# CurryChen77/RIFT

Measured on AMD Instinct MI355X. Metric: policy-update scenes/sec (256-scene RIFT update steps on a 4096-scene replay), higher is better.
Workload: dtype bf16; 1 GPU; BASELINE configs[2]/[3]: full rift_pluto CBV policy, 4096-scene synthetic replay (64 agents x 21 steps, 20 polygons x 3 x 20 pts, R~U{1..6} x 120 ref pts, 12 modes), RIFT loss, pi_head trainable; per_gpu_batch=256, global_batch=256, replay_scenes_per_gpu=4096, parallelism=dp1, train_mode=dropout+droppath+state-dropout, BN batch stats

## Files before the change

rift_amd/csrc/engine.hip:

```cpp
#include <hip/hip_runtime.h>
#include <math.h>
#include <stdio.h>
#include <stdlib.h>
#include <string.h>

#include <set>
#include <cmath>
#include <string>
#include <unordered_map>
#include <dlfcn.h>
#include <vector>

#include "../../include/rift_hip.h"
#include "adv.h"
#include "gemm.h"
#include "kernels.h"
#include "loss.h"
#include "nat_l0w.h"
#include "nat_l1w.h"
#include "enc_fused.h"
#include "enc_fused.h"
#include "dec_w.h"
#include "dec_kv.h"
#include "nat_l2w.h"
#include "enc_w.h"
#include "pe_w.h"
#include "fo_w.h"
#include "pe_fused.h"
#include "fourier_fused.h"
#include "critic.h"
#include "fpn_fused.h"
#include "ego_fused.h"
#include "front.h"
#include "heads_fused.h"
#include "pi_fused.h"
#include "rollout.h"
#include "tick_multi.h"

#define ENC_NW 8

using namespace RIFT_NS;

namespace {

struct Param { void* data; int64_t numel; int ndim; int64_t shape[4]; };

struct PW {
  void* bf = nullptr; float* f32 = nullptr; const float* bias = nullptr;
  int N = 0, K = 0, Kp = 0, Npad = 0;
  void* hid = nullptr;
};

struct Tap { float* p; int64_t numel; };

}

struct RiftCtx {
  int opfmt = 0;
  int device = 0;
  std::string err;
  std::unordered_map<std::string, Param> params;
  std::unordered_map<std::string, PW> pw;
  std::vector<void*> owned;
  struct WConst { float* p = nullptr; bool ready = false; };
// ... 12 lines not shown
  float* ro_raw = nullptr; size_t ro_cap = 0;
  char* tick_scratch = nullptr; size_t tick_cap = 0;
  bool dry = false;
  hipStream_t stream = nullptr;
  std::unordered_map<std::string, Tap> taps;
  float* last_qfinal = nullptr; float* last_hpi = nullptr; float* last_prob = nullptr;
  uint8_t* last_rkpm = nullptr; int last_bs = 0, last_R = 0;
  double* l_S = nullptr; double* l_cnt = nullptr; float* l_dz = nullptr; float* l_partial = nullptr;
  size_t l_cap_bs = 0, l_cap_rows = 0, l_cap_wg = 0;
  float* ego_w = nullptr; float* ego_b = nullptr;
  bool nat_fused = true; int gemm_dbg = 0;
  unsigned short* l0w_img = nullptr; float* l0w_par = nullptr;
  unsigned short* encw_img = nullptr; float* encw_par = nullptr;
  unsigned short* l2w_img = nullptr; float* l2w_par = nullptr;
  unsigned short* l1w_img = nullptr; float* l1w_par = nullptr;
  unsigned short* enc_wqkv[4] = {nullptr, nullptr, nullptr, nullptr};
  float* enc_bqkv[4] = {nullptr, nullptr, nullptr, nullptr};
  int* enc_idx = nullptr; bool enc_fused = true;
  int poison_lds = -1;
  struct { std::string delay_label; long long delay_ticks = 0; int pe_ts = -1, pew_dbg = 0, pew_ts = 0, nat_ts = 0, enc_ts = 0, dec_ts = 0, dec_dbg = 0, poison_arena = -1; } dg;
  hipEvent_t param_event = nullptr;
  bool dec_fused = true;
  bool two_streams = true; bool nat_on_main = true; bool nat_compact = true; bool pe_live = true; bool pe_pack = true; bool tok_fused = false; bool keep_tokens = false; bool front_fused = false; bool front_ego = false; bool ego_nofit = false;
  hipStream_t prep_stream = nullptr; bool prep_set = false; hipEvent_t ev_prep = nullptr; int side_gate = 0;
  hipEvent_t ev_join2 = nullptr; bool nat_aside = true; int join_once = -1;
  hipStream_t side = nullptr; bool side_owned = false; hipEvent_t ev_fork = nullptr, ev_join = nullptr;
  bool fo_w = true; unsigned short* fow_img[3] = {nullptr, nullptr, nullptr}; float* fow_par[3] = {nullptr, nullptr, nullptr};
  bool pe_w = true; unsigned short* pew_img[2] = {nullptr, nullptr};
  unsigned short* decw_img = nullptr; float* decw_par = nullptr;
  double* clip_part = nullptr;
  struct Dp { bool on = false; int off = 0, gbs = 0; double* xchg = nullptr; long long len = 0; RiftExchangeFn fn = nullptr; void* user = nullptr; } dp;
  int* nonfinite = nullptr;
  unsigned long long* rk_pub[RIFT_DEFER_SLOTS] = {}; int rk_cap[RIFT_DEFER_SLOTS] = {}; unsigned int rk_epoch[RIFT_DEFER_SLOTS] = {};
  bool rank_fault = false;
  bool enc112 = true;
  bool rank_in_prep = true;
  void* comm = nullptr; int comm_rank = 0, comm_world = 1;
  float* cr_buf = nullptr; size_t cr_cap = 0; double* cr_part = nullptr;
  bool pe_fused = true; bool fo_fused = true; int nat_grid = 256; bool fpn_fused = true; bool ego_fused = true; bool heads_fused = true; bool pi_fused = true;
  bool loaded = false;
  bool prof_on = false; double prof_flops = 0.0; bool prof_shapes = false;
  std::set<std::string> prof_names;
  std::vector<hipEvent_t> prof_pool; size_t prof_used = 0;
  struct Rec { const char* label; hipEvent_t e0, e1; double flops; };
  std::vector<Rec> prof_recs;
};

static void prof_events(RiftCtx* c, hipEvent_t* e0, hipEvent_t* e1) {
  while (c->prof_pool.size() < c->prof_used + 2) { hipEvent_t e; (void)hipEventCreate(&e); c->prof_pool.push_back(e); }
  *e0 = c->prof_pool[c->prof_used++]; *e1 = c->prof_pool[c->prof_used++];
}
static void prof_push(RiftCtx* c, const char* label, hipEvent_t e0, hipEvent_t e1, double flops) {
  c->prof_recs.push_back(RiftCtx::Rec{label, e0, e1, flops});
}

#define HIPCHK(ctx, expr)                                                                 \
  do {                                                                                    \
    hipError_t e__ = (expr);                                                              \
    if (e__ != hipSuccess) {                                                              \
      (ctx)->err = std::string(#expr) + ": " + hipGetErrorString(e__);                    \
      return RIFT_ERR_HIP;                                                                \
    }                                                                                     \
  } while (0)

namespace {

// ... 702 lines not shown
    g.gbias = h.x0p; g.gb_div = R * M; g.gb_mod = 0;
    gemm(c, g, c->pw[PD + ".cat_x_proj.q"], h.fp32);
    PW w; w.N = 128; w.K = 128; w.Kp = 128; w.Npad = 128;
    w.f32 = (float*)fptr(c, PD + ".pi_head.mlp.0.weight"); w.bias = fptr(c, PD + ".pi_head.mlp.0.bias");
    gemm(c, mk(h.QF, 128, nQ, w, h.Hpi, 128), w, true);
    launch(c, "pi_tail_kernel", pi_tail_kernel, dim3(cdiv(nQ, 4)), dim3(256), 0, (const float*)h.Hpi, nQ, M, fptr(c, PD + ".pi_head.mlp.1.weight"),
           fptr(c, PD + ".pi_head.mlp.1.bias"), fptr(c, PD + ".pi_head.mlp.3.weight"), fptr(c, PD + ".pi_head.mlp.3.bias"),
           (const uint8_t*)h.r_kpm, 1e-5f, h.prob, c->nonfinite);
  }
  tap(c, "q_final", h.QF, (int64_t)nQ * 128);
  if (h.need_traj && !h.fp32 && c->heads_fused) {
    const std::string nm3[3] = {PD + ".loc_head", PD + ".yaw_head", PD + ".vel_head"};
    heads3_fused(f, h.QF, 128, nQ, 0, 0, 0, nm3, h.traj);
  } else if (h.need_traj) {
    const char* nm[3] = {"loc_head", "yaw_head", "vel_head"};
    for (int i = 0; i < 3; ++i) {
      const PW& w0 = c->pw[PD + "." + nm[i] + ".mlp.0"];
      const PW& w3 = c->pw[PD + "." + nm[i] + ".mlp.3"];
      float* T = h.oT[i];
      gemm(c, mk(h.QF, 128, nQ, w0, T, w0.N), w0, h.fp32);
      GemmP g = mk(T, w0.N, nQ, w3, h.o3[i], 160);
      g.pro = PRO_LN; g.pg = fptr(c, PD + "." + nm[i] + ".mlp.1.weight"); g.pb = fptr(c, PD + "." + nm[i] + ".mlp.1.bias"); g.pro_relu = 1;
      gemm(c, g, w3, h.fp32);
    }
    launch(c, "interleave_traj_kernel", interleave_traj_kernel, dim3(cdiv((long long)nQ * 480, 256)), dim3(256), 0, (const float*)h.o3[0], (const float*)h.o3[1],
           (const float*)h.o3[2], nQ, h.traj);
  }
  if (!c->dry) {
    c->last_qfinal = h.QF; c->last_hpi = h.Hpi; c->last_prob = h.prob; c->last_rkpm = h.r_kpm; c->last_bs = h.bs; c->last_R = h.R;
  }
  return RIFT_OK;
}

int forward_impl(RiftCtx* c, const RiftFeatureBatch* B, const RiftOutputs* out, int flags, uint32_t seed) {
  Fwd f;
  f.c = c; f.train = (flags & RIFT_F_TRAIN) != 0; f.drop = f.train && !(flags & RIFT_F_NO_DROP);
  f.fp32 = (flags & RIFT_F_FP32) != 0; f.need_traj = (flags & RIFT_F_NEED_TRAJ) != 0;
  f.bn_update = f.train && !(flags & RIFT_F_NO_BN_UPDATE); f.seed = seed;
  const int bs = B->bs, A = B->A, Mp = B->Mp, R = B->R, S = B->S, T = B->T;
  const int N = A + Mp + S, M = 12;
  const int nA = bs * A, nP = bs * Mp, nL = bs * R, nQ = nL * M, nT = bs * N;
  const std::string HE = "agent_encoder.history_encoder";

  (void)A_alloc<float>(c, 64);
  float* F9 = A_alloc<float>(c, (size_t)nA * 20 * 9 + 64);
  uint8_t* valid_agent = A_alloc<uint8_t>(c, nA);
  const bool nat_compact = c->nat_compact && c->nat_fused && !f.fp32 && c->fpn_fused;
  uint8_t* hist_agent = nat_compact ? A_alloc<uint8_t>(c, nA) : nullptr;
  int* nat_aidx = nat_compact ? A_alloc<int>(c, nA) : nullptr;
  int* nat_cnt = nat_compact ? A_alloc<int>(c, 4) : nullptr;
  float* F10 = A_alloc<float>(c, (size_t)nP * 20 * 10);
  float* F6 = A_alloc<float>(c, (size_t)nL * 120 * 6);
  uint8_t* kpm = A_alloc<uint8_t>(c, nT);
  float* pos = A_alloc<float>(c, (size_t)nT * 3);
  float* r_pos = A_alloc<float>(c, (size_t)nL * 3);
  uint8_t* r_kpm = A_alloc<uint8_t>(c, nL);
  bool prefetched = false;
  bool front_fused = false; float* x_ego_front = nullptr; EgoP ego_front; memset(&ego_front, 0, sizeof(ego_front));
  f.r_tiles = A_alloc<uint8_t>(c, (size_t)std::max(nL, 1));
  {
    PrepP q; memset(&q, 0, sizeof(q));
    q.agent_pos = B->agent_position; q.agent_head = B->agent_heading; q.agent_vel = B->agent_velocity; q.agent_shape = B->agent_shape;
    q.agent_valid = B->agent_valid_mask; q.nA = nA; q.Tfull = T; q.F9 = F9; q.valid_agent = valid_agent; q.hist_agent = hist_agent;
    q.map_pp = B->map_point_position; q.map_pv = B->map_point_vector; q.map_po = B->map_point_orientation; q.map_center = B->map_polygon_center;
    q.nPoly = nP; q.F10 = F10;
    q.ref_pos = B->ref_position; q.ref_vec = B->ref_vector; q.ref_ori = B->ref_orientation; q.ref_valid = B->ref_valid_mask; q.nLine = nL;
    q.F6 = F6; q.r_pos = r_pos; q.r_kpm = r_kpm; q.r_tiles = f.r_tiles;
    q.map_valid = B->map_valid_mask; q.static_valid = B->static_valid_mask; q.st_pos = B->static_position; q.st_head = B->static_heading;
    q.bs = bs; q.A = A; q.Mp = Mp; q.S = S; q.kpm = kpm; q.pos = pos;
    q.nb[0] = cdiv((long long)nA * 20, 256); q.nb[1] = cdiv((long long)nP * 20, 256); q.nb[2] = cdiv((long long)nL * 120, 256);
    q.nb[3] = cdiv(nL, 256); q.nb[4] = cdiv(nL, 256); q.nb[5] = cdiv(nT, 256); q.nb[6] = cdiv(nT, 256);
    int tot = 0;
    for (int i = 0; i < 7; ++i) tot += q.nb[i];
    const bool rank_in_prep = nat_compact && c->rank_in_prep && A <= 256 && !(c->front_fused && !f.fp32 && c->ego_fused);
    if (rank_in_prep) {
      const int sl = c->parity;
      if (c->rk_cap[sl] < bs) {
        HIPCHK(c, hipDeviceSynchronize());
        if (c->rk_pub[sl]) { HIPCHK(c, hipFree(c->rk_pub[sl])); c->rk_pub[sl] = nullptr; c->rk_cap[sl] = 0; }
        const int cap = std::max(2 * bs, 4096);
        HIPCHK(c, hipMalloc((void**)&c->rk_pub[sl], (size_t)cap * sizeof(unsigned long long)));
        HIPCHK(c, hipMemset(c->rk_pub[sl], 0, (size_t)cap * sizeof(unsigned long long)));
        HIPCHK(c, hipDeviceSynchronize());
        c->rk_cap[sl] = cap; c->rk_epoch[sl] = 0;
      }
      q.nrk = bs; q.rk_pub = c->rk_pub[sl]; q.aidx = nat_aidx; q.cnt = nat_cnt; q.fail = c->nonfinite; q.rk_fault = c->rank_fault ? 1 : 0;
      if (!c->dry) { if (++c->rk_epoch[sl] == 0u) c->rk_epoch[sl] = 1u; }
      q.rk_epoch = c->rk_epoch[sl];
      q.hist_agent = nullptr;
      tot += bs;
    }
    front_fused = c->front_fused && !f.fp32 && c->ego_fused && !RIFT_DROP_STATS;
    FrontP fq; memset(&fq, 0, sizeof(fq));
    if (front_fused) {
      const std::string EG = "agent_encoder.ego_state_emb";
      bool fill_eq;
      float* eq = wconst_get(c, "ego_q", 128, f.fp32, &fill_eq);
      if (fill_eq) gemm(c, mk(fptr(c, EG + ".query"), 128, 1, c->pw[EG + ".attn.q"], eq, 128), c->pw[EG + ".attn.q"], f.fp32);
      x_ego_front = A_alloc<float>(c, (size_t)bs * 128);
      EgoP& e = fq.ego;
      e.cs = B->current_state; e.cs_ld = B->cs_ld; e.lw = c->ego_w; e.lb = c->ego_b; e.pos = fptr(c, EG + ".pos_embed");
      e.wkv = (const unsigned short*)c->pw[EG + ".attn.kv"].bf; e.bkv = c->pw[EG + ".attn.kv"].bias; e.q = eq;
      e.wo = (const unsigned short*)c->pw[EG + ".attn.out_proj"].bf; e.bo = c->pw[EG + ".attn.out_proj"].bias;
      e.out = x_ego_front; e.bs = bs; e.drop_p = f.drop ? 0.75f : 0.f; e.seed = f.seed; e.stream = 0x45474Fu;
      ego_front = e;
      fq.n_ego = c->front_ego ? bs : 0;
      fq.rank_on = nat_compact ? 1 : 0; fq.aidx = nat_aidx; fq.cnt = nat_cnt;
      if (nat_compact) q.hist_agent = nullptr;
      fq.prep = q;
    }
    auto launch_front = [&]() {
      if (front_fused) {
        c->prof_flops = 2.0 * bs * (6.0 * 128 * 256 + 128.0 * 128);
        if (fq.n_ego) launch(c, "front_kernel", front_kernel<true>, dim3(tot + fq.n_ego + fq.rank_on), dim3(256), 0, fq);
        else launch(c, "front_kernel", front_kernel<false>, dim3(tot + fq.rank_on), dim3(256), 0, fq);
      } else {
        launch(c, "prep_kernel", prep_kernel, dim3(tot), dim3(256), 0, q);
        if (nat_compact && !rank_in_prep) launch(c, "nat_rank_kernel", nat_rank_kernel, dim3(1), dim3(NAT_RANK_THREADS), 0, (const uint8_t*)hist_agent, nA, nat_aidx, nat_cnt);
      }
    };
    prefetched = c->prep_set && !c->prof_on && !c->dry;
    if (prefetched) {
      if (!c->ev_prep) HIPCHK(c, hipEventCreateWithFlags(&c->ev_prep, hipEventDisableTiming));
      hipStream_t own = c->stream;
      c->stream = c->prep_stream;
      launch_front();
      c->stream = own;
      HIPCHK(c, hipEventRecord(c->ev_prep, c->prep_stream));
      const bool join_covers = c->two_streams && c->nat_fused && !f.fp32 && c->nat_aside && c->side_gate <= 0 && !c->dp.on;
      if (!join_covers) HIPCHK(c, hipStreamWaitEvent(own, c->ev_prep, 0));
    } else {
      launch_front();
    }
  }
  const uint8_t* q_kpm = r_kpm; int q_bs = bs, q_off = 0;
  if (c->dp.on) {
    f.dp = true; f.kb = c->dp.gbs * R; f.kpm_pending = true;
    f.g_rkpm = A_alloc<uint8_t>(c, (size_t)f.kb);
    if ((long long)f.kb + 2 * 513 > c->dp.len || c->dp.off < 0 || c->dp.off + bs > c->dp.gbs) { c->err = "rift_set_dp: exchange buffer too small or shard outside the global minibatch"; return RIFT_ERR_ARG; }
    if (!prefetched) launch(c, "dp_kpm_fill_kernel", dp_kpm_fill_kernel, dim3(cdiv(f.kb, 256)), dim3(256), 0, (const uint8_t*)r_kpm, nL, c->dp.off * R, f.kb, c->dp.xchg);
    q_kpm = f.g_rkpm; q_bs = c->dp.gbs; q_off = c->dp.off;
  }
  const bool dp_fill_late = c->dp.on && prefetched;
#if RIFT_DROP_STATS
  DropStats ds; memset(&ds, 0, sizeof(ds));
  if (f.drop) {
    ds.nmax = std::max(nA, bs * 6);
    const size_t n = (size_t)RIFT_DS_SITES * ds.nmax;
    ds.cnt = A_alloc<unsigned int>(c, n); ds.any = A_alloc<unsigned int>(c, n); ds.all = A_alloc<unsigned int>(c, n);
    ds.scale = A_alloc<float>(c, RIFT_DS_SITES + RIFT_DS_DEC_SITES); ds.elem = A_alloc<unsigned long long>(c, 2 * RIFT_DS_DEC_SITES);
    if (!c->dry) {
      HIPCHK(c, hipMemsetAsync(ds.cnt, 0, n * 4, c->stream)); HIPCHK(c, hipMemsetAsync(ds.any, 0, n * 4, c->stream));
      HIPCHK(c, hipMemsetAsync(ds.all, 0xff, n * 4, c->stream));
      HIPCHK(c, hipMemsetAsync(ds.scale, 0, (RIFT_DS_SITES + RIFT_DS_DEC_SITES) * 4, c->stream));
      HIPCHK(c, hipMemsetAsync(ds.elem, 0, 2 * RIFT_DS_DEC_SITES * 8, c->stream));
    }
    tap(c, "drop_cnt", (float*)ds.cnt, (int64_t)n); tap(c, "drop_any", (float*)ds.any, (int64_t)n); tap(c, "drop_all", (float*)ds.all, (int64_t)n);
    tap(c, "drop_scale", ds.scale, RIFT_DS_SITES + RIFT_DS_DEC_SITES); tap(c, "drop_elem", (float*)ds.elem, 4 * RIFT_DS_DEC_SITES);
  }
#define RIFT_SET_DS(x) (x).ds = ds
#else
#define RIFT_SET_DS(x)
#endif
  if (nat_compact) { tap(c, "nat_aidx", (float*)nat_aidx, nA); tap(c, "nat_cnt", (float*)nat_cnt, 3); }
  static const float dpr[6] = {0.f, 0.04f, 0.08f, 0.12f, 0.16f, 0.2f};
  const bool fused = c->nat_fused && !f.fp32;
  hipStream_t main_stream = c->stream;
  const bool forked = c->two_streams && fused && !c->prof_on && !c->dry;
  bool nat_aside = false;
  if (forked) {
    if (!c->side) { HIPCHK(c, hipStreamCreateWithFlags(&c->side, hipStreamNonBlocking)); c->side_owned = true; }
    if (!c->ev_fork) { HIPCHK(c, hipEventCreateWithFlags(&c->ev_fork, hipEventDisableTiming)); HIPCHK(c, hipEventCreateWithFlags(&c->ev_join, hipEventDisableTiming)); }
    const bool gate = c->side_gate > 0;
    if (prefetched) HIPCHK(c, hipStreamWaitEvent(c->side, c->ev_prep, 0));
    if (!prefetched || gate) {
      HIPCHK(c, hipEventRecord(c->ev_fork, main_stream));
      HIPCHK(c, hipStreamWaitEvent(c->side, c->ev_fork, 0));
    }
    nat_aside = prefetched && !gate && c->nat_aside;
    if (nat_aside) {
      if (!c->ev_join2) HIPCHK(c, hipEventCreateWithFlags(&c->ev_join2, hipEventDisableTiming));
      c->stream = c->prep_stream;
    } else if (!c->nat_on_main) c->stream = c->side;
  }
  static const int Ll[3] = {20, 10, 5}, Cl[3] = {32, 64, 128}, Hl[3] = {2, 4, 8}, Kl[3] = {3, 3, 5};
  float* Oc[3];
  for (int i = 0; i < 3; ++i) Oc[i] = A_alloc<float>(c, (size_t)nA * 3 * Cl[i]);
  const bool oc_bf16 = fused && c->fpn_fused;
  unsigned short* Ocb[3] = {nullptr, nullptr, nullptr};
  if (oc_bf16) for (int i = 0; i < 3; ++i) Ocb[i] = A_alloc<unsigned short>(c, (size_t)nA * 3 * Cl[i]);
  if (fused) {
    float* Xin[3] = {nullptr, A_alloc<float>(c, (size_t)nA * 10 * 64), A_alloc<float>(c, (size_t)nA * 5 * 128)};
    for (int lv = 0; lv < 3; ++lv) {
      const int C = Cl[lv], H = Hl[lv], ksz = Kl[lv], L = Ll[lv], rows = nA * L;
      if (lv == 0) {
        NatL0WP q; memset(&q, 0, sizeof(q));
        q.aidx = nat_aidx; q.cnt = nat_cnt;
        q.F9 = F9; q.nseq = nA; q.img = c->l0w_img; q.par = c->l0w_par; q.Oc = Oc[0]; q.Ocb = Ocb[0]; q.Xnext = Xin[1];
        { if (c->dg.nat_ts == 1) { q.ts = A_alloc<long long>(c, 64); tap(c, "nat_ts", (float*)q.ts, 128); } }
        q.droppath[0] = f.drop ? dpr[0] : 0.f; q.droppath[1] = f.drop ? dpr[1] : 0.f; q.seed = f.seed; q.stream = f.next_stream(); f.stream_id += 4;
        RIFT_SET_DS(q);
        c->prof_flops = 2.0 * rows * (20.0 * C * C + 4.0 * ksz * C) + 2.0 * rows * 27 * 32 + (rows / 2) * 2.0 * 3 * C * 2 * C;
        { const int g0 = std::min(cdiv(cdiv(nA, 4), L0W_NWV), c->nat_grid); launch_call(c, "nat_l0w_kernel", [&] { l0w_launch(q, g0, c->stream); }); }
        continue;
      }
      if (lv == 1) {
        NatL1WP q; memset(&q, 0, sizeof(q));
        q.cnt = nat_cnt;
        q.X = Xin[1]; q.nseq = nA; q.img = c->l1w_img; q.par = c->l1w_par; q.Oc = Oc[1]; q.Ocb = Ocb[1]; q.Xnext = Xin[2];
        q.droppath[0] = f.drop ? dpr[2] : 0.f; q.droppath[1] = f.drop ? dpr[3] : 0.f; q.seed = f.seed; q.stream = f.next_stream(); f.stream_id += 4;
        RIFT_SET_DS(q);
        c->prof_flops = 2.0 * rows * (20.0 * C * C + 4.0 * ksz * C) + (rows / 2) * 2.0 * 3 * C * 2 * C;
        { const int g1 = std::min(cdiv(cdiv(nA, 4), L1W_NWV), c->nat_grid); launch_call(c, "nat_l1w_kernel", [&] { l1w_launch(q, g1, c->stream); }); }
        continue;
      }
// ... 18 lines not shown
      gemm(c, g, c->pw[HE + ".embed.proj"], f.fp32);
    }
    auto nat_level = [&](float* Xl, int lv, int rows, int C, int H, int ksz, int L) {
      nat_layer(f, Xl, rows, C, H, ksz, L, HE + ".levels." + std::to_string(lv) + ".blocks.0", dpr[2 * lv]);
      nat_layer(f, Xl, rows, C, H, ksz, L, HE + ".levels." + std::to_string(lv) + ".blocks.1", dpr[2 * lv + 1]);
    };
    nat_level(X0, 0, nA * 20, 32, 2, 3, 20);
    float* X1 = A_alloc<float>(c, (size_t)nA * 10 * 64);
    {
      GemmP g = mk(X0, 32, nA * 10, c->pw[HE + ".levels.0.downsample.reduction"], X1, 64);
      g.amode = AMODE_CONV3; g.cv_C = 32; g.cv_Lin = 20; g.cv_nout = 10; g.cv_t0 = 0; g.cv_stride = 2;
      gemm(c, g, c->pw[HE + ".levels.0.downsample.reduction"], f.fp32);
      layernorm(f, X1, 64, X1, 64, nA * 10, 64, HE + ".levels.0.downsample.norm");
    }
    nat_level(X1, 1, nA * 10, 64, 4, 3, 10);
    float* X2 = A_alloc<float>(c, (size_t)nA * 5 * 128);
    {
      GemmP g = mk(X1, 64, nA * 5, c->pw[HE + ".levels.1.downsample.reduction"], X2, 128);
      g.amode = AMODE_CONV3; g.cv_C = 64; g.cv_Lin = 10; g.cv_nout = 5; g.cv_t0 = 0; g.cv_stride = 2;
      gemm(c, g, c->pw[HE + ".levels.1.downsample.reduction"], f.fp32);
      layernorm(f, X2, 128, X2, 128, nA * 5, 128, HE + ".levels.1.downsample.norm");
    }
    nat_level(X2, 2, nA * 5, 128, 8, 5, 5);
    tap(c, "nat_level2", X2, (int64_t)nA * 5 * 128);
    float* Xl[3] = {X0, X1, X2};
    for (int i = 0; i < 3; ++i)
      for (int j = 0; j < 3; ++j)
        launch(c, "layernorm_kernel", layernorm_kernel, dim3(cdiv(nA, 4)), dim3(256), 0, (const float*)(Xl[i] + (size_t)(Ll[i] - 3 + j) * Cl[i]),
               Ll[i] * Cl[i], Oc[i] + (size_t)j * Cl[i], 3 * Cl[i], nA, Cl[i],
               fptr(c, HE + ".norm" + std::to_string(i) + ".weight"), fptr(c, HE + ".norm" + std::to_string(i) + ".bias"),
               1e-5f, 0);
  }
  float* nat_out = A_alloc<float>(c, (size_t)nA * 128);
  if (fused && c->fpn_fused) {
    FpnP q; memset(&q, 0, sizeof(q));
    for (int i = 0; i < 3; ++i) {
      const PW& w = c->pw[HE + ".lateral_convs." + std::to_string(i)];
      q.oc[i] = Oc[i]; q.ocb[i] = Ocb[i]; q.wl[i] = (const unsigned short*)w.bf; q.bl[i] = w.bias;
    }
    q.wf = (const unsigned short*)c->pw[HE + ".fpn_conv.last"].bf; q.bf_ = c->pw[HE + ".fpn_conv.last"].bias;
    q.out = nat_out; q.nA = nA; q.cnt = fused ? nat_cnt : nullptr; q.aidx = fused ? nat_aidx : nullptr;
    c->prof_flops = 2.0 * nA * (2.0 * 128 * (96 + 192 + 384) + 256.0 * 128);
    launch(c, "fpn_tail_kernel", fpn_tail_kernel, dim3(cdiv(nA, FPN_AG)), dim3(512), (size_t)FPN_LDS, q);
  } else {
    float* lat[3];
    for (int i = 0; i < 3; ++i) {
      lat[i] = A_alloc<float>(c, (size_t)nA * 2 * 128);
      const std::string lc = HE + ".lateral_convs." + std::to_string(i);
      GemmP g = mk(Oc[i], Cl[i], nA * 2, c->pw[lc], lat[i], 128);
      g.amode = AMODE_CONV3; g.cv_C = Cl[i]; g.cv_Lin = 3; g.cv_nout = 2; g.cv_t0 = 1; g.cv_stride = 1;
      gemm(c, g, c->pw[lc], f.fp32);
    }
    float* Z = A_alloc<float>(c, (size_t)nA * 256);
    launch(c, "fpn_merge_kernel", fpn_merge_kernel, dim3(cdiv((long long)nA * 128, 256)), dim3(256), 0, (const float*)lat[0], (const float*)lat[1],
           (const float*)lat[2], nA, Z);
    gemm(c, mk(Z, 256, nA, c->pw[HE + ".fpn_conv.last"], nat_out, 128), c->pw[HE + ".fpn_conv.last"], f.fp32);
  }
  if (forked) {
    if (nat_aside) { HIPCHK(c, hipEventRecord(c->ev_join2, c->prep_stream)); c->stream = c->side; }
    else if (c->nat_on_main) c->stream = c->side;
    else { HIPCHK(c, hipEventRecord(c->ev_join, c->side)); c->stream = main_stream; }
  }
  if (dp_fill_late)
    launch(c, "dp_kpm_fill_kernel", dp_kpm_fill_kernel, dim3(cdiv(f.kb, 256)), dim3(256), 0, (const uint8_t*)r_kpm, nL, c->dp.off * R, f.kb, c->dp.xchg);
  tap(c, "nat_out", nat_out, (int64_t)nA * 128);

  const std::string EG = "agent_encoder.ego_state_emb";
  bool fill_eq;
  float* eq = wconst_get(c, "ego_q", 128, f.fp32, &fill_eq);
  if (fill_eq) gemm(c, mk(fptr(c, EG + ".query"), 128, 1, c->pw[EG + ".attn.q"], eq, 128), c->pw[EG + ".attn.q"], f.fp32);
  float* x_ego = front_fused ? x_ego_front : A_alloc<float>(c, (size_t)bs * 128);
  if (front_fused && c->front_ego) {
    if (f.drop) (void)f.next_stream();
  } else if (!f.fp32 && c->ego_fused) {
    EgoP q; memset(&q, 0, sizeof(q));
    if (front_fused) { q = ego_front; q.stream = f.drop ? f.next_stream() : 0; } else {
    q.cs = B->current_state; q.cs_ld = B->cs_ld; q.lw = c->ego_w; q.lb = c->ego_b; q.pos = fptr(c, EG + ".pos_embed");
    q.wkv = (const unsigned short*)c->pw[EG + ".attn.kv"].bf; q.bkv = c->pw[EG + ".attn.kv"].bias; q.q = eq;
    q.wo = (const unsigned short*)c->pw[EG + ".attn.out_proj"].bf; q.bo = c->pw[EG + ".attn.out_proj"].bias;
    q.out = x_ego; q.bs = bs; q.drop_p = f.drop ? 0.75f : 0.f; q.seed = f.seed; q.stream = f.drop ? f.next_stream() : 0;
    }
    RIFT_SET_DS(q);
    c->prof_flops = 2.0 * bs * (6.0 * 128 * 256 + 128.0 * 128);
    launch(c, "ego_fused_kernel", ego_fused_kernel, dim3(bs), dim3(256), (size_t)(c->ego_nofit ? 40960 : 0), q);
  } else {
  float* E = A_alloc<float>(c, (size_t)bs * 6 * 128);
  launch(c, "ego_token_kernel", ego_token_kernel, dim3(cdiv((long long)bs * 6 * 128, 256)), dim3(256), 0, B->current_state, B->cs_ld,
         (const float*)c->ego_w, (const float*)c->ego_b, fptr(c, EG + ".pos_embed"), bs, E);
  float* EKV = A_alloc<float>(c, (size_t)bs * 6 * 256);
  gemm(c, mk(E, 128, bs * 6, c->pw[EG + ".attn.kv"], EKV, 256), c->pw[EG + ".attn.kv"], f.fp32);
  uint8_t* edrop = nullptr;
  if (f.drop) {
// ... 36 lines not shown
      w.count = 3;
      for (int i = 0; i < 3; ++i) {
        const FourierP& o = q3.e[i]; FoWSide& d = w.e[i];
        d.in = o.in; d.in_ld = o.in_ld; d.rows = o.rows; d.D = o.D; d.wrap_dim = o.wrap_dim; d.img = c->fow_img[i]; d.par = c->fow_par[i];
        d.Y = o.Y; d.accumulate = o.accumulate; d.rep = o.D == 1 ? 2 : 1; d.nwg = cdiv(cdiv(o.rows, 16), 8 * d.rep);
      }
      launch_call(c, "fo_w_kernel", [&] { fow_launch(w, c->stream); });
    } else
    launch(c, "fourier_fused_kernel", fourier_fused_kernel, dim3(q3.nblk[0] + q3.nblk[1] + q3.nblk[2]), dim3(256), (size_t)FO_LDS, q3);
    PEtok = q3.e[0].Y; speed_emb = q3.e[1].Y; rpe_done = true;
  } else {
    speed_emb = fourier(f, B->map_polygon_speed_limit, 1, nP, 1, "map_encoder.speed_limit_emb", -1);
  }
  float* Q = nullptr;
  auto build_q0 = [&]() -> int {
  bool fill;
  float* Mb = wconst_get(c, "Mb", (size_t)M * 128, f.fp32, &fill);
  if (fill) gemm(c, mk(fptr(c, PD + ".m_emb"), 128, M, c->pw[PD + ".q_proj.m"], Mb, 128), c->pw[PD + ".q_proj.m"], f.fp32);
  Q = A_alloc<float>(c, (size_t)nQ * 128);
  if (!f.fp32 && c->pi_fused) {
    Q0P q; memset(&q, 0, sizeof(q));
    q.r_emb = r_emb; q.nL = nL; q.M = M; q.wr = (const unsigned short*)c->pw[PD + ".q_proj.r"].bf; q.br = c->pw[PD + ".q_proj.r"].bias;
    q.Mb = Mb; q.Q = Q;
    c->prof_flops = 2.0 * nL * 128.0 * 128;
    launch(c, "q0_fused_kernel", q0_fused_kernel, dim3(cdiv(nL, 16)), dim3(256), 0, q);
  } else {
    float* Ra = A_alloc<float>(c, (size_t)nL * 128);
    gemm(c, mk(r_emb, 128, nL, c->pw[PD + ".q_proj.r"], Ra, 128), c->pw[PD + ".q_proj.r"], f.fp32);
    launch(c, "build_q0_kernel", build_q0_kernel, dim3(cdiv((long long)nQ * 128, 256)), dim3(256), 0, (const float*)Ra, (const float*)Mb, nL, M, Q);
  }
    return RIFT_OK;
  };
  if (forked && rpe_done) { const int rc0 = build_q0(); if (rc0 != RIFT_OK) return rc0; }
  const bool join_once = nat_aside && (c->join_once >= 0 ? c->join_once != 0 : bs <= 64);
  if (join_once) HIPCHK(c, hipStreamWaitEvent(c->side, c->ev_join2, 0));
  if (forked && (c->nat_on_main || nat_aside)) { HIPCHK(c, hipEventRecord(c->ev_join, c->side)); c->stream = main_stream; }
  if (forked) HIPCHK(c, hipStreamWaitEvent(main_stream, c->ev_join, 0));
  if (nat_aside && !join_once) HIPCHK(c, hipStreamWaitEvent(main_stream, c->ev_join2, 0));
  const bool tok_fused = c->tok_fused && c->enc_fused && !f.fp32 && N <= 96 && S == 0 && fo3 && PEtok != nullptr;
  TokenP tokq; memset(&tokq, 0, sizeof(tokq));
  {
    TokenP& q = tokq;
    q.nat = nat_out; q.x_ego = x_ego; q.valid_agent = (const uint8_t*)valid_agent; q.category = B->agent_category; q.a_type_emb = fptr(c, "agent_encoder.type_emb.weight");
    q.pooled = poly; q.ptype = B->map_polygon_type; q.on_route = B->map_polygon_on_route; q.tl = B->map_polygon_tl_status; q.has_sl = B->map_polygon_has_speed_limit;
    q.speed_emb = speed_emb; q.p_type_emb = fptr(c, "map_encoder.type_emb.weight"); q.route_emb = fptr(c, "map_encoder.on_route_emb.weight");
    q.tl_emb = fptr(c, "map_encoder.traffic_light_emb.weight"); q.unk_emb = fptr(c, "map_encoder.unknown_speed_emb.weight");
    q.bs = bs; q.A = A; q.Mp = Mp; q.N = N; q.X = X; q.pe = PEtok;
    q.nblk_a = cdiv((long long)nA * 32, 256);
    if (!tok_fused) launch(c, "token_kernel", token_kernel, dim3(q.nblk_a + cdiv((long long)nP * 32, 256)), dim3(256), 0, q);
  }
  if (S > 0) {
    float* semb = fourier(f, B->static_shape, 2, bs * S, 2, "static_objects_encoder.obj_encoder", -1);
    launch(c, "static_token_kernel", static_token_kernel, dim3(cdiv((long long)bs * S * 128, 256)), dim3(256), 0, (const float*)semb, B->static_category,
           B->static_valid_mask, fptr(c, "static_objects_encoder.type_emb.weight"), bs, A, Mp, S, N, X);
  }
  if (!fo3) fourier(f, pos, 3, nT, 3, "pos_emb", 2, X);
  tap(c, "x_tokens", X, (int64_t)nT * 128);

  static const float edpr[4] = {0.f, 0.2f / 3.f, 0.4f / 3.f, 0.2f};
  float* ENC = A_alloc<float>(c, (size_t)nT * 128);
  unsigned short* enc_KT = nullptr;
  uint8_t* kpm_c = nullptr;
  float* enc_x0p = nullptr;
  const bool enc_wide = N > 96 && N <= 112 && c->enc112 && c->dec_fused && R <= 8 && ENC_NW == 8 && !tok_fused;
  if (c->enc_fused && !f.fp32 && (N <= 96 || enc_wide)) {
    EncFusedP ep; memset(&ep, 0, sizeof(ep));
    ep.X = X; ep.Y = ENC; ep.kpm = kpm; ep.bs = bs; ep.N = N; ep.seed = f.seed; ep.stream = f.next_stream(); f.stream_id += 8;
    if (tok_fused) { ep.tok = tokq; ep.tok_on = 1; ep.Xout = c->keep_tokens ? X : nullptr; }
    for (int i = 0; i < 4; ++i) {
      const std::string p = "encoder_blocks." + std::to_string(i);
      EncBlockW& w = ep.blk[i];
// ... 86 lines not shown
  }

  if (!pe_pair) r_emb = points_encoder(f, F6, 6, nL, 120, B->ref_valid_mask, PD + ".r_encoder");
  if (!rpe_done) {
    tap(c, "r_pe", r_emb, (int64_t)nL * 128);
    fourier(f, r_pos, 3, nL, 3, PD + ".r_pos_emb", -1, r_emb);
  }
  tap(c, "r_emb", r_emb, (int64_t)nL * 128);
  if (!Q) { const int rc0 = build_q0(); if (rc0 != RIFT_OK) return rc0; }
  tap(c, "q0", Q, (int64_t)nQ * 128);

  bool dec_deferred = false; DecWP dec_later; memset(&dec_later, 0, sizeof(dec_later));
  dp_exchange(f, 0);
  const float dp = f.drop ? 0.1f : 0.f;
  const bool dec_dense = (R > 8 || N > 96) && R <= 16 && N <= 192;
  if (c->dec_fused && !f.fp32 && dec_dense && !enc_KT) {
    enc_KT = A_alloc<unsigned short>(c, (size_t)bs * 4 * 96 * 512);
    DecKvP kq; memset(&kq, 0, sizeof(kq));
    kq.ENC = ENC; kq.bs = bs; kq.N = N; kq.wkv = (const unsigned short*)c->pw[PD + ".kv_all"].bf; kq.bkv = c->pw[PD + ".kv_all"].bias; kq.KV = enc_KT;
    c->prof_flops = 2.0 * bs * N * 128.0 * 1024;
    launch(c, "dec_kv_frag_kernel", dec_kv_frag_kernel, dim3(bs), dim3(512), (size_t)DEC_KV_LDS, kq);
  }
  if (c->dec_fused && !f.fp32 && ((R <= 8 && N <= 96) || dec_dense) && enc_KT) {
    DecWP dq; memset(&dq, 0, sizeof(dq));
    dq.Q = Q; dq.kpm = kpm; dq.r_kpm = r_kpm; dq.q_kpm = q_kpm; dq.q_bs = q_bs; dq.q_off = q_off; dq.bs = bs; dq.N = N; dq.R = R; dq.dropout = dp; dq.seed = f.seed;
    if (kpm_c) { dq.kpm = kpm_c; dq.N = enc_wide ? 112 : 96; dq.compact = 1; }
    dq.stream = f.next_stream(); f.stream_id += 64;
    dq.KV = enc_KT; dq.img = c->decw_img; dq.par = c->decw_par; dq.nonfinite = c->nonfinite;
    RIFT_SET_DS(dq);
    if (c->dg.dec_ts) { dq.ts = A_alloc<long long>(c, 1024); tap(c, "dec_ts", (float*)dq.ts, 2048); }
    dq.dbg = c->dg.dec_dbg;
    c->prof_flops = 4.0 * bs * (R * M) * (2.0 * 128 * (384 + 128) * 2 + 2.0 * 128 * 128 * 2 + 4.0 * 128 * 512 + 4.0 * 128 * (N + R + M));
    dq.l0 = 0; dq.l1 = 4;
    const bool dec_size_ok = c->dec_defer_max >= 0 ? bs <= c->dec_defer_max : (f.need_traj ? bs <= 128 : (bs <= 84 || (bs >= 108 && bs <= 192)));
    const bool dec_may_defer = (flags & RIFT_F_DEFER_HEAD) && dec_size_ok && !c->prof_on;
    uint32_t* rng_io = (dec_may_defer && c->dec_split && !f.need_traj) ? A_alloc<uint32_t>(c, (size_t)bs * 512 * 4) : nullptr;
    dec_deferred = dec_may_defer && !c->dry && !dq.ts;
    if (dec_deferred) {
      dec_later = dq;
      if (rng_io) {
        dq.l1 = 2; dq.rng_io = rng_io;
        launch_call(c, "dec_w_kernel", [&] { decw_launch(dq, c->stream); });
        dec_later.l0 = 2; dec_later.rng_io = rng_io;
      }
    } else launch_call(c, "dec_w_kernel", [&] { decw_launch(dq, c->stream); });
  } else {
  float* DQKV = A_alloc<float>(c, (size_t)nQ * 384);
  float* DAO = A_alloc<float>(c, (size_t)nQ * 128);
  float* DQc = A_alloc<float>(c, (size_t)nQ * 128);
  float* DH = A_alloc<float>(c, (size_t)nQ * 512);
  float* KVm = A_alloc<float>(c, (size_t)nT * 256);
  float* MP = A_alloc<float>(c, (size_t)M * 384);
  for (int i = 0; i < 4; ++i) {
    const std::string p = PD + ".decoder_blocks." + std::to_string(i);
    GemmP g = mk(Q, 128, nQ, c->pw[p + ".r2r_attn.qkv"], DQKV, 384);
    g.pro = PRO_LN; g.pg = fptr(c, p + ".norm1.weight"); g.pb = fptr(c, p + ".norm1.bias");
    gemm(c, g, c->pw[p + ".r2r_attn.qkv"], f.fp32);
    {
      MhaP m; memset(&m, 0, sizeof(m));
      m.Q = DQKV; m.ldq = 384; m.K = DQKV + 128; m.V = DQKV + 256; m.ldkv = 384; m.O = DAO; m.ldo = 128;
      m.nb_outer = bs; m.nb_inner = M; m.H = 4; m.Lq = R; m.Lk = R;
      m.q_outer = R * M; m.q_inner = 1; m.q_stride = M; m.kv_outer = R * M; m.kv_inner = 1; m.kv_stride = M;
      m.o_outer = R * M; m.o_inner = 1; m.o_stride = M;
      m.mask = q_kpm; m.mask_quirk = 1; m.mask_mod = q_bs; m.mask_off = q_off * M;
      if (dp > 0.f) { m.dropout_p = dp; m.seed = f.seed; m.stream = f.next_stream(); }
      run_mha(c, m, f.fp32);
    }
    GemmP g2 = mk(DAO, 128, nQ, c->pw[p + ".r2r_attn.out_proj"], Q, 128);
// ... 93 lines not shown

namespace RIFT_NS { namespace abi {

int rift_ctx_create(int device, RiftCtx** ctx) {
  if (!ctx) return RIFT_ERR_ARG;
  RiftCtx* c = new RiftCtx();
  c->opfmt = RIFT_OP_F16;
  c->device = device;
  if (hipSetDevice(device) != hipSuccess) { delete c; return RIFT_ERR_HIP; }
  { const char* ev = getenv("RIFT_NAT_UNFUSED"); c->nat_fused = !(ev && ev[0] == '1'); }
  { const char* ev = getenv("RIFT_DEC_UNFUSED"); c->dec_fused = !(ev && ev[0] == '1'); }
  { const char* ev = getenv("RIFT_ENC_UNFUSED"); c->enc_fused = !(ev && ev[0] == '1'); }
  { const char* ev = getenv("RIFT_PE_UNFUSED"); c->pe_fused = !(ev && ev[0] == '1'); }
  { const char* ev = getenv("RIFT_FPN_UNFUSED"); c->fpn_fused = !(ev && ev[0] == '1'); }
  { const char* ev = getenv("RIFT_EGO_UNFUSED"); c->ego_fused = !(ev && ev[0] == '1'); }
  { const char* ev = getenv("RIFT_HEADS_UNFUSED"); c->heads_fused = !(ev && ev[0] == '1'); }
  { const char* ev = getenv("RIFT_PI_UNFUSED"); c->pi_fused = !(ev && ev[0] == '1'); }
  { const char* ev = getenv("RIFT_NAT_GRID"); if (ev && atoi(ev) > 0) c->nat_grid = atoi(ev); }
  { const char* ev = getenv("RIFT_NAT_MAIN"); if (ev) c->nat_on_main = atoi(ev) != 0; }
  { const char* ev = getenv("RIFT_NAT_COMPACT"); if (ev) c->nat_compact = atoi(ev) != 0; }
  { const char* ev = getenv("RIFT_PE_LIVE"); if (ev) c->pe_live = atoi(ev) != 0; }
  { const char* ev = getenv("RIFT_PE_PACK"); if (ev) c->pe_pack = atoi(ev) != 0; }
  { const char* ev = getenv("RIFT_TOKEN_FUSED"); if (ev) c->tok_fused = atoi(ev) != 0; }
  { const char* ev = getenv("RIFT_KEEP_TOKENS"); c->keep_tokens = ev && ev[0] == '1'; }
  { const char* ev = getenv("RIFT_FRONT_FUSED"); if (ev) c->front_fused = atoi(ev) != 0; }
  { const char* ev = getenv("RIFT_RANK_IN_PREP"); if (ev) c->rank_in_prep = atoi(ev) != 0; }
  { const char* ev = getenv("RIFT_ENC112"); if (ev) c->enc112 = atoi(ev) != 0; }
  { const char* ev = getenv("RIFT_RANK_FAULT"); if (ev) c->rank_fault = atoi(ev) != 0; }
  { const char* ev = getenv("RIFT_EGO_NOFIT"); c->ego_nofit = ev && ev[0] == '1'; }
  { const char* ev = getenv("RIFT_FRONT_EGO"); if (ev) c->front_ego = atoi(ev) != 0; }
  { const char* ev = getenv("RIFT_SIDE_GATE"); if (ev) c->side_gate = atoi(ev); }
  { const char* ev = getenv("RIFT_NAT_ASIDE"); if (ev) c->nat_aside = atoi(ev) != 0; }
  { const char* ev = getenv("RIFT_JOIN_ONCE"); if (ev) c->join_once = atoi(ev); }
  { const char* ev = getenv("RIFT_DEC_DEFER"); if (ev) c->dec_defer_max = atoi(ev); }
  { const char* ev = getenv("RIFT_DEC_SPLIT"); if (ev) c->dec_split = atoi(ev) != 0; }
  { const char* ev = getenv("RIFT_RO8"); if (ev) c->ro8 = atoi(ev) != 0; }
  { const char* ev = getenv("RIFT_POISON_LDS"); if (ev) c->poison_lds = (int)strtol(ev, nullptr, 0) & 0xff; }
  { const char* ev = getenv("RIFT_POISON_ARENA"); if (ev) c->dg.poison_arena = (int)strtol(ev, nullptr, 0) & 0xff; }
  { const char* ev = getenv("RIFT_PE_TS"); if (ev) c->dg.pe_ts = atoi(ev); }
  { const char* ev = getenv("RIFT_DELAY"); const char* col = ev ? strrchr(ev, ':') : nullptr;
    if (col) { c->dg.delay_label.assign(ev, col - ev); c->dg.delay_ticks = (long long)(atof(col + 1) * 100.0); } }
  { const char* ev = getenv("RIFT_PEW_DBG"); if (ev) c->dg.pew_dbg = atoi(ev); }
  { const char* ev = getenv("RIFT_PEW_TS"); c->dg.pew_ts = ev && ev[0] == '1'; }
  { const char* ev = getenv("RIFT_NAT_TS"); if (ev) c->dg.nat_ts = atoi(ev); }
  c->dg.enc_ts = getenv("RIFT_ENC_TS") != nullptr; c->dg.dec_ts = getenv("RIFT_DEC_TS") != nullptr;
  { const char* ev = getenv("RIFT_DEC_DBG"); if (ev) c->dg.dec_dbg = atoi(ev); }
  { const char* ev = getenv("RIFT_FOURIER_UNFUSED"); c->fo_fused = !(ev && ev[0] == '1'); }
  { const char* ev = getenv("RIFT_PE_W"); c->pe_w = !(ev && ev[0] == '0'); }
  { const char* ev = getenv("RIFT_FO_W"); c->fo_w = !(ev && ev[0] == '0'); }
  { const char* ev = getenv("RIFT_TWO_STREAMS"); c->two_streams = !(ev && ev[0] == '0'); }
  { const char* ev = getenv("RIFT_GEMM_DBG"); c->gemm_dbg = ev ? atoi(ev) : 0; }
  if (hipMalloc((void**)&c->nonfinite, sizeof(int)) != hipSuccess || hipMemset(c->nonfinite, 0, sizeof(int)) != hipSuccess) { delete c; return RIFT_ERR_HIP; }
  for (int i = 0; i < RIFT_DEFER_SLOTS; ++i) {
    if (hipMalloc((void**)&c->rk_pub[i], 4096 * sizeof(unsigned long long)) != hipSuccess || hipMemset(c->rk_pub[i], 0, 4096 * sizeof(unsigned long long)) != hipSuccess) { delete c; return RIFT_ERR_HIP; }
    c->rk_cap[i] = 4096;
  }
  if (hipDeviceSynchronize() != hipSuccess) { delete c; return RIFT_ERR_HIP; }
  int rc = set_lds_attrs(c);
  if (rc != RIFT_OK) { fprintf(stderr, "rift_ctx_create: %s\n", c->err.c_str()); delete c; return rc; }
  *ctx = c;
  return RIFT_OK;
}

void rift_ctx_destroy(RiftCtx* c) {
  if (!c) return;
  if (c->comm) { (void)rccl_api(nullptr).CommDestroy(c->comm); c->comm = nullptr; }
  if (c->tick_scratch) (void)hipFree(c->tick_scratch);
  if (c->ro_raw) (void)hipFree(c->ro_raw);
  for (void* p : c->owned) (void)hipFree(p);
  for (int i = 0; i < RIFT_DEFER_SLOTS; ++i) if (c->arenas[i]) (void)hipFree(c->arenas[i]);
  if (c->l_S) (void)hipFree(c->l_S);
  if (c->l_cnt) (void)hipFree(c->l_cnt);
  if (c->l_dz) (void)hipFree(c->l_dz);
  if (c->l_partial) (void)hipFree(c->l_partial);
  if (c->ego_w) (void)hipFree(c->ego_w);
  if (c->ego_b) (void)hipFree(c->ego_b);
  if (c->enc_idx) (void)hipFree(c->enc_idx);
  if (c->cr_buf) { (void)hipFree(c->cr_buf); (void)hipFree(c->cr_part); }
  if (c->clip_part) (void)hipFree(c->clip_part);
  if (c->nonfinite) (void)hipFree(c->nonfinite);
  for (int i = 0; i < RIFT_DEFER_SLOTS; ++i) if (c->rk_pub[i]) (void)hipFree(c->rk_pub[i]);
  if (c->l0w_img) { (void)hipFree(c->l0w_img); (void)hipFree(c->l0w_par); }
  if (c->l1w_img) { (void)hipFree(c->l1w_img); (void)hipFree(c->l1w_par); }
  if (c->l2w_img) { (void)hipFree(c->l2w_img); (void)hipFree(c->l2w_par); }
  if (c->encw_img) { (void)hipFree(c->encw_img); (void)hipFree(c->encw_par); }
  if (c->decw_img) { (void)hipFree(c->decw_img); (void)hipFree(c->decw_par); }
  for (int i = 0; i < 2; ++i) if (c->pew_img[i]) (void)hipFree(c->pew_img[i]);
  for (int i = 0; i < 3; ++i) if (c->fow_img[i]) { (void)hipFree(c->fow_img[i]); (void)hipFree(c->fow_par[i]); }
  if (c->ev_prep) (void)hipEventDestroy(c->ev_prep);
  if (c->ev_join2) (void)hipEventDestroy(c->ev_join2);
  if (c->side && c->side_owned) (void)hipStreamDestroy(c->side);
  if (c->ev_fork) { (void)hipEventDestroy(c->ev_fork); (void)hipEventDestroy(c->ev_join); }
  for (int i = 0; i < 4; ++i) { if (c->enc_wqkv[i]) (void)hipFree(c->enc_wqkv[i]); if (c->enc_bqkv[i]) (void)hipFree(c->enc_bqkv[i]); }
  delete c;
}

const char* rift_last_error(RiftCtx* c) { return c ? c->err.c_str() : "null context"; }

int rift_model_load(RiftCtx* c, const RiftTensorDesc* params, int n, void* stream) {
  if (!c || !params) return RIFT_ERR_ARG;
  c->err.clear();
  c->stream = (hipStream_t)stream;
  HIPCHK(c, hipSetDevice(c->device));
  for (void* p : c->owned) (void)hipFree(p);
  c->owned.clear(); c->pw.clear(); c->params.clear(); c->wconst.clear();
  c->dry_need = 0;
  for (int i = 0; i < n; ++i) {
    Param p; p.data = params[i].data; p.numel = params[i].numel; p.ndim = params[i].ndim;
    for (int d = 0; d < 4; ++d) p.shape[d] = params[i].shape[d];
    c->params[params[i].name] = p;
  }
  const std::string HE = "agent_encoder.history_encoder";
  TRY(pack_conv(c, HE + ".embed.proj"));
  for (int lv = 0; lv < 3; ++lv) {
// ... 921 lines not shown
```

Before: 461,100 scenes/s.

## Defer FPN tail past stream join and guard ranking slot reuse across streams

Adds a 'chain' schedule for large batches (bs>192): the FPN tail kernel is launched on the main stream after the NAT/map streams join instead of at the end of the NAT stream, with an optional swap of which stream carries NAT vs map work. It also adds per-slot events tracking which stream last used a ranking publication slot, ordering or refusing reuse across streams, and reuses that event as the prep-done event. The intent is to shorten the critical path on the side streams and improve overlap, at the cost of extra event bookkeeping and a moved kernel that may now serialize on main.

Result: no change. 465,100 scenes/s, median of 6 (+0.9%).

```diff
diff --git a/rift_amd/csrc/engine.hip b/rift_amd/csrc/engine.hip
--- a/rift_amd/csrc/engine.hip
+++ b/rift_amd/csrc/engine.hip
@@ -30,6 +30,7 @@
 #include "fourier_fused.h"
 #include "critic.h"
 #include "fpn_fused.h"
+#include "rk_guard.h"
 #include "ego_fused.h"
 #include "front.h"
 #include "heads_fused.h"
@@ -108,6 +109,8 @@
   struct Dp { bool on = false; int off = 0, gbs = 0; double* xchg = nullptr; long long len = 0; RiftExchangeFn fn = nullptr; void* user = nullptr; } dp;
   int* nonfinite = nullptr;
   unsigned long long* rk_pub[RIFT_DEFER_SLOTS] = {}; int rk_cap[RIFT_DEFER_SLOTS] = {}; unsigned int rk_epoch[RIFT_DEFER_SLOTS] = {};
+  hipEvent_t rk_ev[RIFT_DEFER_SLOTS] = {}; hipStream_t rk_stream[RIFT_DEFER_SLOTS] = {}; bool rk_armed[RIFT_DEFER_SLOTS] = {};
+  int chain_sched = 1;
   bool rank_fault = false;
   bool enc112 = true;
   bool rank_in_prep = true;
@@ -876,6 +879,10 @@
   return RIFT_OK;
 }
 
+static bool dec_defer_size(const RiftCtx* c, int bs, bool need_traj) {
+  return c->dec_defer_max >= 0 ? bs <= c->dec_defer_max : (need_traj ? bs <= 128 : (bs <= 84 || (bs >= 108 && bs <= 192)));
+}
+
 int forward_impl(RiftCtx* c, const RiftFeatureBatch* B, const RiftOutputs* out, int flags, uint32_t seed) {
   Fwd f;
   f.c = c; f.train = (flags & RIFT_F_TRAIN) != 0; f.drop = f.train && !(flags & RIFT_F_NO_DROP);
@@ -885,6 +892,15 @@
   const int N = A + Mp + S, M = 12;
   const int nA = bs * A, nP = bs * Mp, nL = bs * R, nQ = nL * M, nT = bs * N;
   const std::string HE = "agent_encoder.history_encoder";
+  const bool fused = c->nat_fused && !f.fp32;
+  const bool prefetched = c->prep_set && !c->prof_on && !c->dry;
+  const bool forked = c->two_streams && fused && !c->prof_on && !c->dry;
+  const bool nat_aside = forked && prefetched && c->side_gate <= 0 && c->nat_aside;
+  const bool join_once = nat_aside && (c->join_once >= 0 ? c->join_once != 0 : bs <= 64);
+  const bool dec_may_defer = (flags & RIFT_F_DEFER_HEAD) && dec_defer_size(c, bs, f.need_traj) && !c->prof_on;
+  const bool chain = nat_aside && !join_once && c->chain_sched > 0 && c->fpn_fused && !c->dp.on && !dec_may_defer && bs > 192;
+  const bool chain_swap = chain && c->chain_sched == 2;
+  hipStream_t nat_st = chain_swap ? c->side : c->prep_stream, map_st = chain_swap ? c->prep_stream : c->side;
 
   (void)A_alloc<float>(c, 64);
   float* F9 = A_alloc<float>(c, (size_t)nA * 20 * 9 + 64);
@@ -899,7 +915,7 @@
   float* pos = A_alloc<float>(c, (size_t)nT * 3);
   float* r_pos = A_alloc<float>(c, (size_t)nL * 3);
   uint8_t* r_kpm = A_alloc<uint8_t>(c, nL);
-  bool prefetched = false;
+  hipEvent_t prep_ev = nullptr;
   bool front_fused = false; float* x_ego_front = nullptr; EgoP ego_front; memset(&ego_front, 0, sizeof(ego_front));
   f.r_tiles = A_alloc<uint8_t>(c, (size_t)std::max(nL, 1));
   {
@@ -928,6 +944,19 @@
         HIPCHK(c, hipDeviceSynchronize());
         c->rk_cap[sl] = cap; c->rk_epoch[sl] = 0;
       }
+      if (!c->dry) {
+        const hipStream_t ls = prefetched ? c->prep_stream : c->stream;
+        int st = 1;
+        if (c->rk_armed[sl] && c->rk_stream[sl] != ls) {
+          const hipError_t qe = c->rk_ev[sl] ? hipEventQuery(c->rk_ev[sl]) : hipErrorInvalidResourceHandle;
+          st = qe == hipSuccess ? 1 : (qe == hipErrorNotReady ? 0 : -1);
+        }
+        const rk_guard::Verdict v = rk_guard::slot_verdict(c->rk_stream[sl], c->rk_armed[sl], st, ls);
+        if (v == rk_guard::RK_REFUSE) { c->err = "forward: the ranking slot's last launch may still be in flight on another stream"; return RIFT_ERR_ARG; }
+        if (v == rk_guard::RK_ORDER) HIPCHK(c, hipStreamWaitEvent(ls, c->rk_ev[sl], 0));
+        if (!c->rk_ev[sl]) HIPCHK(c, hipEventCreateWithFlags(&c->rk_ev[sl], hipEventDisableTiming));
+        c->rk_stream[sl] = ls; c->rk_armed[sl] = true;
+      }
       q.nrk = bs; q.rk_pub = c->rk_pub[sl]; q.aidx = nat_aidx; q.cnt = nat_cnt; q.fail = c->nonfinite; q.rk_fault = c->rank_fault ? 1 : 0;
       if (!c->dry) { if (++c->rk_epoch[sl] == 0u) c->rk_epoch[sl] = 1u; }
       q.rk_epoch = c->rk_epoch[sl];
@@ -963,18 +992,20 @@
         if (nat_compact && !rank_in_prep) launch(c, "nat_rank_kernel", nat_rank_kernel, dim3(1), dim3(NAT_RANK_THREADS), 0, (const uint8_t*)hist_agent, nA, nat_aidx, nat_cnt);
       }
     };
-    prefetched = c->prep_set && !c->prof_on && !c->dry;
+    const int rk_sl = rank_in_prep && !c->dry ? c->parity : -1;
     if (prefetched) {
       if (!c->ev_prep) HIPCHK(c, hipEventCreateWithFlags(&c->ev_prep, hipEventDisableTiming));
+      prep_ev = rk_sl >= 0 ? c->rk_ev[rk_sl] : c->ev_prep;
       hipStream_t own = c->stream;
       c->stream = c->prep_stream;
       launch_front();
       c->stream = own;
-      HIPCHK(c, hipEventRecord(c->ev_prep, c->prep_stream));
-      const bool join_covers = c->two_streams && c->nat_fused && !f.fp32 && c->nat_aside && c->side_gate <= 0 && !c->dp.on;
-      if (!join_covers) HIPCHK(c, hipStreamWaitEvent(own, c->ev_prep, 0));
+      HIPCHK(c, hipEventRecord(prep_ev, c->prep_stream));
+      const bool join_covers = nat_aside && !c->dp.on;
+      if (!join_covers) HIPCHK(c, hipStreamWaitEvent(own, prep_ev, 0));
     } else {
       launch_front();
+      if (rk_sl >= 0) HIPCHK(c, hipEventRecord(c->rk_ev[rk_sl], c->stream));
     }
   }
   const uint8_t* q_kpm = r_kpm; int q_bs = bs, q_off = 0;
@@ -1008,23 +1039,19 @@
 #endif
   if (nat_compact) { tap(c, "nat_aidx", (float*)nat_aidx, nA); tap(c, "nat_cnt", (float*)nat_cnt, 3); }
   static const float dpr[6] = {0.f, 0.04f, 0.08f, 0.12f, 0.16f, 0.2f};
-  const bool fused = c->nat_fused && !f.fp32;
   hipStream_t main_stream = c->stream;
-  const bool forked = c->two_streams && fused && !c->prof_on && !c->dry;
-  bool nat_aside = false;
   if (forked) {
     if (!c->side) { HIPCHK(c, hipStreamCreateWithFlags(&c->side, hipStreamNonBlocking)); c->side_owned = true; }
     if (!c->ev_fork) { HIPCHK(c, hipEventCreateWithFlags(&c->ev_fork, hipEventDisableTiming)); HIPCHK(c, hipEventCreateWithFlags(&c->ev_join, hipEventDisableTiming)); }
     const bool gate = c->side_gate > 0;
-    if (prefetched) HIPCHK(c, hipStreamWaitEvent(c->side, c->ev_prep, 0));
+    if (prefetched) HIPCHK(c, hipStreamWaitEvent(c->side, prep_ev, 0));
     if (!prefetched || gate) {
       HIPCHK(c, hipEventRecord(c->ev_fork, main_stream));
       HIPCHK(c, hipStreamWaitEvent(c->side, c->ev_fork, 0));
     }
-    nat_aside = prefetched && !gate && c->nat_aside;
     if (nat_aside) {
       if (!c->ev_join2) HIPCHK(c, hipEventCreateWithFlags(&c->ev_join2, hipEventDisableTiming));
-      c->stream = c->prep_stream;
+      c->stream = nat_st;
     } else if (!c->nat_on_main) c->stream = c->side;
   }
   static const int Ll[3] = {20, 10, 5}, Cl[3] = {32, 64, 128}, Hl[3] = {2, 4, 8}, Kl[3] = {3, 3, 5};
@@ -1109,16 +1136,20 @@
                1e-5f, 0);
   }
   float* nat_out = A_alloc<float>(c, (size_t)nA * 128);
+  FpnP fpn_q; memset(&fpn_q, 0, sizeof(fpn_q));
+  auto launch_fpn = [&]() {
+    c->prof_flops = 2.0 * nA * (2.0 * 128 * (96 + 192 + 384) + 256.0 * 128);
+    launch(c, "fpn_tail_kernel", fpn_tail_kernel, dim3(cdiv(nA, FPN_AG)), dim3(512), (size_t)FPN_LDS, fpn_q);
+  };
   if (fused && c->fpn_fused) {
-    FpnP q; memset(&q, 0, sizeof(q));
+    FpnP& q = fpn_q;
     for (int i = 0; i < 3; ++i) {
       const PW& w = c->pw[HE + ".lateral_convs." + std::to_string(i)];
       q.oc[i] = Oc[i]; q.ocb[i] = Ocb[i]; q.wl[i] = (const unsigned short*)w.bf; q.bl[i] = w.bias;
     }
     q.wf = (const unsigned short*)c->pw[HE + ".fpn_conv.last"].bf; q.bf_ = c->pw[HE + ".fpn_conv.last"].bias;
     q.out = nat_out; q.nA = nA; q.cnt = fused ? nat_cnt : nullptr; q.aidx = fused ? nat_aidx : nullptr;
-    c->prof_flops = 2.0 * nA * (2.0 * 128 * (96 + 192 + 384) + 256.0 * 128);
-    launch(c, "fpn_tail_kernel", fpn_tail_kernel, dim3(cdiv(nA, FPN_AG)), dim3(512), (size_t)FPN_LDS, q);
+    if (!chain) launch_fpn();
   } else {
     float* lat[3];
     for (int i = 0; i < 3; ++i) {
@@ -1134,7 +1165,7 @@
     gemm(c, mk(Z, 256, nA, c->pw[HE + ".fpn_conv.last"], nat_out, 128), c->pw[HE + ".fpn_conv.last"], f.fp32);
   }
   if (forked) {
-    if (nat_aside) { HIPCHK(c, hipEventRecord(c->ev_join2, c->prep_stream)); c->stream = c->side; }
+    if (nat_aside) { HIPCHK(c, hipEventRecord(c->ev_join2, nat_st)); c->stream = map_st; }
     else if (c->nat_on_main) c->stream = c->side;
     else { HIPCHK(c, hipEventRecord(c->ev_join, c->side)); c->stream = main_stream; }
   }
@@ -1237,11 +1268,11 @@
     return RIFT_OK;
   };
   if (forked && rpe_done) { const int rc0 = build_q0(); if (rc0 != RIFT_OK) return rc0; }
-  const bool join_once = nat_aside && (c->join_once >= 0 ? c->join_once != 0 : bs <= 64);
   if (join_once) HIPCHK(c, hipStreamWaitEvent(c->side, c->ev_join2, 0));
-  if (forked && (c->nat_on_main || nat_aside)) { HIPCHK(c, hipEventRecord(c->ev_join, c->side)); c->stream = main_stream; }
+  if (forked && (c->nat_on_main || nat_aside)) { HIPCHK(c, hipEventRecord(c->ev_join, nat_aside ? map_st : c->side)); c->stream = main_stream; }
   if (forked) HIPCHK(c, hipStreamWaitEvent(main_stream, c->ev_join, 0));
   if (nat_aside && !join_once) HIPCHK(c, hipStreamWaitEvent(main_stream, c->ev_join2, 0));
+  if (chain) launch_fpn();
   const bool tok_fused = c->tok_fused && c->enc_fused && !f.fp32 && N <= 96 && S == 0 && fo3 && PEtok != nullptr;
   TokenP tokq; memset(&tokq, 0, sizeof(tokq));
   {
@@ -1394,8 +1425,6 @@
     dq.dbg = c->dg.dec_dbg;
     c->prof_flops = 4.0 * bs * (R * M) * (2.0 * 128 * (384 + 128) * 2 + 2.0 * 128 * 128 * 2 + 4.0 * 128 * 512 + 4.0 * 128 * (N + R + M));
     dq.l0 = 0; dq.l1 = 4;
-    const bool dec_size_ok = c->dec_defer_max >= 0 ? bs <= c->dec_defer_max : (f.need_traj ? bs <= 128 : (bs <= 84 || (bs >= 108 && bs <= 192)));
-    const bool dec_may_defer = (flags & RIFT_F_DEFER_HEAD) && dec_size_ok && !c->prof_on;
     uint32_t* rng_io = (dec_may_defer && c->dec_split && !f.need_traj) ? A_alloc<uint32_t>(c, (size_t)bs * 512 * 4) : nullptr;
     dec_deferred = dec_may_defer && !c->dry && !dq.ts;
     if (dec_deferred) {
@@ -1555,6 +1584,7 @@
   { const char* ev = getenv("RIFT_SIDE_GATE"); if (ev) c->side_gate = atoi(ev); }
   { const char* ev = getenv("RIFT_NAT_ASIDE"); if (ev) c->nat_aside = atoi(ev) != 0; }
   { const char* ev = getenv("RIFT_JOIN_ONCE"); if (ev) c->join_once = atoi(ev); }
+  { const char* ev = getenv("RIFT_CHAIN_SCHED"); if (ev) c->chain_sched = atoi(ev); }
   { const char* ev = getenv("RIFT_DEC_DEFER"); if (ev) c->dec_defer_max = atoi(ev); }
   { const char* ev = getenv("RIFT_DEC_SPLIT"); if (ev) c->dec_split = atoi(ev) != 0; }
   { const char* ev = getenv("RIFT_RO8"); if (ev) c->ro8 = atoi(ev) != 0; }
@@ -1602,7 +1632,7 @@
   if (c->cr_buf) { (void)hipFree(c->cr_buf); (void)hipFree(c->cr_part); }
   if (c->clip_part) (void)hipFree(c->clip_part);
   if (c->nonfinite) (void)hipFree(c->nonfinite);
-  for (int i = 0; i < RIFT_DEFER_SLOTS; ++i) if (c->rk_pub[i]) (void)hipFree(c->rk_pub[i]);
+  for (int i = 0; i < RIFT_DEFER_SLOTS; ++i) { if (c->rk_pub[i]) (void)hipFree(c->rk_pub[i]); if (c->rk_ev[i]) (void)hipEventDestroy(c->rk_ev[i]); }
   if (c->l0w_img) { (void)hipFree(c->l0w_img); (void)hipFree(c->l0w_par); }
   if (c->l1w_img) { (void)hipFree(c->l1w_img); (void)hipFree(c->l1w_par); }
   if (c->l2w_img) { (void)hipFree(c->l2w_img); (void)hipFree(c->l2w_par); }
diff --git a/rift_amd/csrc/rk_guard.h b/rift_amd/csrc/rk_guard.h
--- /dev/null
+++ b/rift_amd/csrc/rk_guard.h
@@ -0,0 +1,12 @@
+#pragma once
+
+namespace rk_guard {
+
+enum Verdict { RK_OK = 0, RK_ORDER = 1, RK_REFUSE = -1 };
+
+inline Verdict slot_verdict(const void* prev_stream, bool armed, int prev_state, const void* stream) {
+  if (!armed || prev_stream == stream || prev_state == 1) return RK_OK;
+  return prev_state == 0 ? RK_ORDER : RK_REFUSE;
+}
+
+}
```
